# anxingle/AlphaPig

Hardware: AMD Instinct MI355X
Metric: self-play games/sec (15x15, n_playout=400) (higher is better)
Workload: dtype f32 (split operands on the bf16/fp16 matrix pipe, fp32 accumulate; <=1e-4 vs float64 oracle)

## Files before the change

### alphapig_amd/csrc/trunk15_wino3h16.h

```cpp
#pragma once
#include <hip/hip_runtime.h>

#include <cmath>
#include <cstdint>
#include <type_traits>

#include "trunk15_wino3h.h"

namespace apz {

struct Wino3H16 {
    static constexpr int C = 128, CK = 16, NCHUNK = C / CK;
    static constexpr int GPLANE = 240;
    static constexpr int VTERM = 32 * 32, VPOS = 2 * VTERM, V_BYTES = 36 * VPOS;
    static constexpr int UNIT = 2 * 32 * 16;
    static constexpr size_t UPK_BYTES = (size_t)4 * 4 * NCHUNK * 9 * 2 * UNIT;
    static constexpr int BIAS_FLOATS = 256;
    static constexpr int MQ_FLOATS = 36 * 16 * 32;
    static constexpr int SROW = 20, SPLANE = 16 * SROW;
    static constexpr int STG_FLOATS = 8 * 4 * SPLANE;
    static constexpr int LDS_BYTES = 2 * V_BYTES;
    static_assert((MQ_FLOATS + STG_FLOATS) * 4 <= LDS_BYTES, "the epilogue area fits over V");
    static_assert(LDS_BYTES <= 160 * 1024, "LDS");
    static_assert(UPK_BYTES == Wino3H::UPK_BYTES, "same weight buffer as trunk15_wino3h.h");
    __host__ __device__ static size_t upk_offset(int co, int ci, int pos, int term) {
        const int i = pos / 6, k = pos % 6, ri = i / 3, ki = k / 3, p9 = 3 * (i % 3) + (k % 3);
        const int cog = co >> 5, r = co & 31, chunk = ci >> 4, half = (ci >> 3) & 1, w = 2 * ri + ki;
        return ((((size_t)(cog * 4 + w) * NCHUNK + chunk) * 9 + p9) * 2 + term) * UNIT + half * 512 + r * 16 + (ci & 7) * 2;
    }
    static float scale_for(double m) { return Wino3H::scale_for(m); }
};

#ifdef APZ_WINO3H_STAMPS
__device__ unsigned long long apz_wino3h16_stamps[4 * 8 * 12];
#endif

#ifndef APZH16_RING
#define APZH16_RING 3
#endif
#ifndef APZH16_RAW_SLOT
#define APZH16_RAW_SLOT 4
#endif

enum { WINO3H16_PLAIN = 0, WINO3H16_STATS = 1, WINO3H16_DGRAD = 2, WINO3H16_PLAIN_SCALED = 3 };

constexpr int ACT_WINDOW_LOG2 = 4;
constexpr int ACT_EXP_MAX = 100;

inline int act_exponent_for(float m) {
    if (!(m > 0.f)) return 0;
    int ex;
    std::frexp((double)m, &ex);
    const int a = ACT_WINDOW_LOG2 - (ex - 1);
    return a < -ACT_EXP_MAX ? -ACT_EXP_MAX : (a > ACT_EXP_MAX ? ACT_EXP_MAX : a);
}

__device__ __forceinline__ int wino3h16_dgrad_exponent(float m) {
    if (!(m > 0.f)) return 0;
    const int e = (int)((__builtin_bit_cast(unsigned, m) >> 23) & 255u);
    const int a = 134 - e;
    return a < -64 ? -64 : (a > 110 ? 110 : a);
}

template <bool RESID, bool RELU = true, int FORM = WINO3H16_PLAIN>
__global__ __launch_bounds__(512) void trunk15_wino3h16_kernel(const float* __restrict__ in, const void* __restrict__ upk,
                                                               const float* __restrict__ bias, const float* __restrict__ resid,
                                                               float* __restrict__ out, int n, unsigned* __restrict__ flag,
                                                               void* __restrict__ aux, int aux_n) {
    using T = Wino3H16;
    constexpr bool STATS = FORM == WINO3H16_STATS, DGRAD = FORM == WINO3H16_DGRAD, SCALED = FORM == WINO3H16_PLAIN_SCALED;
    static_assert(FORM == WINO3H16_PLAIN || SCALED || !RELU, "the training forms have no ReLU");
    static_assert(!SCALED || RELU, "the scaled form is a self-play form");
    static_assert(!STATS || !RESID, "STATS: bias only");
#ifdef APZ_WINO3H_STAMPS
    unsigned long long st_acc[12] = {0, 0, 0, 0, 0, 0, 0, 0, 0, 0, 0, 0};
    unsigned long long st_t = __builtin_readcyclecounter();
    const unsigned long long st_t0 = st_t, st_r0 = __builtin_amdgcn_s_memrealtime();
#define APZH16_STAMP(ph_)                                             \
    {                                                                 \
        const unsigned long long now_ = __builtin_readcyclecounter(); \
        st_acc[ph_] += now_ - st_t;                                   \
        st_t = now_;                                                  \
    }
#else
#define APZH16_STAMP(ph_)
#endif
    extern __shared__ __attribute__((aligned(16))) float lds[];
    char* vbase = reinterpret_cast<char*>(lds);
    float* mq = lds;
    float* stg = mq + T::MQ_FLOATS;

    const int tid = threadIdx.x, lane = tid & 63;
    const int wave = __builtin_amdgcn_readfirstlane(tid >> 6);

    const int npairs = (n + 1) >> 1, G_ = (int)gridDim.x, b_ = (int)blockIdx.x;
    const bool duo = (G_ & 15) == 0;
    const int pair0 = duo ? ((b_ >> 4) * 8 + (b_ & 7)) : b_;
    const int pstride = duo ? (G_ >> 1) : G_;
    const int h_fix = (b_ >> 3) & 1;
    const int np = pair0 < npairs ? (npairs - pair0 + pstride - 1) / pstride : 0;
    const int nitems = duo ? np : 2 * np;
    if (np == 0) return;
    auto item_pair = [&](int t) { return pair0 + (duo ? t : (t >> 1)) * pstride; };
    auto item_half = [&](int t) { return duo ? h_fix : (t & 1); };

    float xsc = 1.f, xisc = 1.f;
    bool aux_inf = false;
    if constexpr (DGRAD) {
        const float* pm = static_cast<const float*>(aux);
        float m = 0.f;
        for (int i = tid; i < aux_n; i += 512) m = fmaxf(m, fabsf(pm[i]));
#pragma unroll
        for (int off = 32; off > 0; off >>= 1) m = fmaxf(m, __shfl_xor(m, off, 64));
        if (lane == 0) lds[wave] = m;
        __syncthreads();
#pragma unroll
        for (int w = 0; w < 8; w++) m = fmaxf(m, lds[w]);
        const int a = __builtin_amdgcn_readfirstlane(wino3h16_dgrad_exponent(m));
        aux_inf = !(m <= 3.4028234664e38f);
        xsc = __builtin_bit_cast(float, (unsigned)(127 + a) << 23);
        xisc = __builtin_bit_cast(float, (unsigned)(127 - a) << 23);
    }
    if constexpr (SCALED) {
        xsc = __builtin_bit_cast(float, (unsigned)(127 + aux_n) << 23);
        xisc = __builtin_bit_cast(float, (unsigned)(127 - aux_n) << 23);
    }

    const unsigned plane_b = T::GPLANE * 4;
    const unsigned act_bytes = (unsigned)n * T::C * plane_b;
    const __amdgpu_buffer_rsrc_t r_in = __builtin_amdgcn_make_buffer_rsrc(const_cast<float*>(in), 0, act_bytes, 0x00020000);
    const __amdgpu_buffer_rsrc_t r_res =
        __builtin_amdgcn_make_buffer_rsrc(const_cast<float*>(RESID ? resid : in), 0, act_bytes, 0x00020000);
    const __amdgpu_buffer_rsrc_t r_out = __builtin_amdgcn_make_buffer_rsrc(out, 0, act_bytes, 0x00020000);
    const __amdgpu_buffer_rsrc_t r_u =
        __builtin_amdgcn_make_buffer_rsrc(const_cast<void*>(upk), 0, (unsigned)T::UPK_BYTES, 0x00020000);
    const __amdgpu_buffer_rsrc_t r_st =
        __builtin_amdgcn_make_buffer_rsrc(STATS ? aux : out, 0, STATS ? (unsigned)n * T::C * 16u : 0u, 0x00020000);
    auto bload = [](const __amdgpu_buffer_rsrc_t& r, unsigned voff, unsigned soff) {
        return __builtin_bit_cast(f32x4, __builtin_amdgcn_raw_buffer_load_b128(r, voff, soff, 0));
    };
    auto bstore = [](const __amdgpu_buffer_rsrc_t& r, unsigned voff, unsigned soff, const f32x4 v) {
        __builtin_amdgcn_raw_buffer_store_b128(__builtin_bit_cast(u32x4, v), r, voff + soff, 0, 0);
    };

    const int tb = wave & 1, cq = wave >> 1;
    const int ttx = lane & 3, tty = (lane >> 2) & 3, tile = lane & 15, cpl = (lane >> 4) & 1, e = lane >> 5;
    const int chl = 4 * cq + 2 * cpl + e;
    const int cpair = 2 * cq + cpl;
    const int vcol = tb * 16 + tile;
    const int tv_off = vcol * 32 + (((cpair >> 2) ^ ((vcol >> 3) & 1)) * 16) + (cpair & 3) * 4 + e * 3 * T::VPOS;
    const unsigned col16_mask = ttx == 3 ? 0u : 0xffffffffu;
    const float c4l = ttx == 0 ? 0.f : 4.f;
    const unsigned raw_vo = (unsigned)(2 * cpl + e) * plane_b + (unsigned)(tty * 4 * 16 + ttx * 4) * 4;
    const unsigned raw_vo3 = tty == 3 ? 0x80000000u : raw_vo + 3u * 64u;
    f32x4 raw[4];
    auto raw_load = [&](int t, int c) {
        const int bdp = 2 * item_pair(t) + tb;
        const int bd = bdp < n ? bdp : n - 1;
        const unsigned so = (unsigned)(bd * T::C + c * T::CK + 4 * cq) * plane_b;
#pragma unroll
        for (int r = 0; r < 3; r++) raw[r] = bload(r_in, raw_vo + (unsigned)r * 64u, so);
        raw[3] = bload(r_in, raw_vo3, so);
    };

    f32x2 tt[6][2];
    float oo[6];
    auto vpass = [&](int kc) {
        f32x2 x[6];
#pragma unroll
        for (int j = 0; j < 2; j++) {
            const float r3 = raw[3][2 * kc + j], r0 = raw[0][2 * kc + j];
            x[0][j] = __builtin_bit_cast(float, __builtin_amdgcn_update_dpp(0, __builtin_bit_cast(int, r3), 0x114, 0xF, 0xF, true));
            x[5][j] = __builtin_bit_cast(float, __builtin_amdgcn_update_dpp(0, __builtin_bit_cast(int, r0), 0x104, 0xF, 0xF, true));
        }
#pragma unroll
        for (int r = 0; r < 4; r++) x[r + 1] = f32x2{raw[r][2 * kc], raw[r][2 * kc + 1]};
        const f32x2 a = fma2(-4.f, x[2], x[4]), b = fma2(-4.f, x[1], x[3]);
        const f32x2 c = x[4] - x[2], d = x[3] - x[1];
        tt[0][kc] = fma2(4.f, x[0], fma2(-5.f, x[2], x[4]));
        tt[1][kc] = a + b;
        tt[2][kc] = a - b;
        tt[3][kc] = fma2(2.f, d, c);
        tt[4][kc] = fma2(-2.f, d, c);
        tt[5][kc] = fma2(4.f, x[1], fma2(-5.f, x[3], x[5]));
    };
    auto col_pass = [&](int j) {
        const float c3 = tt[j][1][1], c0 = tt[j][0][0];
        const int l = __builtin_amdgcn_mov_dpp(__builtin_bit_cast(int, c3), 0x90, 0xF, 0xF, true);
        const int r = __builtin_amdgcn_mov_dpp(__builtin_bit_cast(int, c0), 0xF9, 0xF, 0xF, true);
        const float v0 = __builtin_bit_cast(float, l), v5 = __builtin_bit_cast(float, (unsigned)r & col16_mask);
        const f32x2 ab = fma2(-4.f, tt[j][0], tt[j][1]);
        const f32x2 dc = tt[j][1] - tt[j][0];
        oo[0] = __builtin_fmaf(c4l, v0, __builtin_fmaf(-5.f, tt[j][0][1], tt[j][1][1]));
        oo[3] = __builtin_fmaf(2.f, dc[0], dc[1]);
        oo[1] = ab[1] + ab[0];
        oo[4] = __builtin_fmaf(-2.f, dc[0], dc[1]);
        oo[2] = ab[1] - ab[0];
        oo[5] = __builtin_fmaf(4.f, tt[j][0][0], __builtin_fmaf(-5.f, tt[j][1][0], v5));
    };
    auto exchange = [&]() {
        asm("s_nop 1\n\tv_permlane32_swap_b32 %0, %3\n\tv_permlane32_swap_b32 %1, %4\n\tv_permlane32_swap_b32 %2, %5"
            : "+v"(oo[0]), "+v"(oo[1]), "+v"(oo[2]), "+v"(oo[3]), "+v"(oo[4]), "+v"(oo[5]));
    };
    auto emit = [&](char* vp, float ev, float od) {
        typedef _Float16 f16x2_ __attribute__((ext_vector_type(2)));
        const f16x2_ h2 = {(_Float16)ev, (_Float16)od};
        const unsigned hu = __builtin_bit_cast(unsigned, h2);
        unsigned lu;
        asm("v_fma_mixlo_f16 %0, %1, -1.0, %2 op_sel:[0,0,0] op_sel_hi:[1,0,0]" : "=v"(lu) : "v"(hu), "v"(ev));
        asm("v_fma_mixhi_f16 %0, %1, -1.0, %2 op_sel:[1,0,0] op_sel_hi:[1,0,0]" : "+v"(lu) : "v"(hu), "v"(od));
        *reinterpret_cast<unsigned*>(vp) = hu;
        *reinterpret_cast<unsigned*>(vp + T::VTERM) = lu;
    };
    auto tslice = [&](int vpar, auto KK) {
        constexpr int K = decltype(KK)::value;
        char* vp = vbase + vpar * T::V_BYTES + tv_off;
        if constexpr ((DGRAD || SCALED) && K == 0) {
#pragma unroll
            for (int r = 0; r < 4; r++) raw[r] *= xsc;
        }
        if constexpr (K < 2) vpass(K);
        else if constexpr (K >= 3) {
            constexpr int j = (K - 3) / 4, part = (K - 3) % 4;
            if constexpr (part == 0) col_pass(j);
            else if constexpr (part == 1) exchange();
            else if constexpr (part == 2) {
                emit(vp + (j * 6 + 0) * T::VPOS, oo[0], oo[3]);
                emit(vp + (j * 6 + 1) * T::VPOS, oo[1], oo[4]);
            } else emit(vp + (j * 6 + 2) * T::VPOS, oo[2], oo[5]);
        }
    };
    auto transform = [&](int vpar) {
#define APZH16_TS(k) tslice(vpar, std::integral_constant<int, k>{});
        APZH16_TS(0) APZH16_TS(1) APZH16_TS(2) APZH16_TS(3) APZH16_TS(4) APZH16_TS(5) APZH16_TS(6) APZH16_TS(7) APZH16_TS(8)
        APZH16_TS(9) APZH16_TS(10) APZH16_TS(11) APZH16_TS(12) APZH16_TS(13) APZH16_TS(14) APZH16_TS(15) APZH16_TS(16)
        APZH16_TS(17) APZH16_TS(18) APZH16_TS(19) APZH16_TS(20) APZH16_TS(21) APZH16_TS(22) APZH16_TS(23) APZH16_TS(24)
        APZH16_TS(25) APZH16_TS(26)
#undef APZH16_TS
    };

    const int cc = wave >> 2, ri = (wave >> 1) & 1, ki = wave & 1, blk = wave & 3;
    const int r31 = lane & 31, hh = lane >> 5;
    const unsigned a_vo = lane * 16;
    const int wpos0 = 18 * ri + 3 * ki;
    auto pos_off = [](int p9) { return (6 * (p9 / 3) + (p9 % 3)) * T::VPOS; };

    static constexpr int RING = APZH16_RING;
    static_assert(18 % RING == 0 && RING >= 2, "ring slots must tile two chunks");
    f16x8 ah[RING], al[RING];
    auto unit_base = [&](int t, int c) {
        const int cog = 2 * item_half(t) + cc;
        return (unsigned)(((cog * 4 + blk) * T::NCHUNK + c) * 18) * T::UNIT;
    };
    unsigned ub_cur = 0, ub_nxt = 0;
    auto unit_pair_at = [&](unsigned base, int p9, int slot) {
        const int u = 2 * p9;
        ah[slot] = __builtin_bit_cast(f16x8, __builtin_amdgcn_raw_buffer_load_b128(r_u, a_vo + (unsigned)(u & 3) * T::UNIT,
                                                                                  base + (unsigned)(u >> 2) * 4u * T::UNIT, 0));
        al[slot] = __builtin_bit_cast(f16x8, __builtin_amdgcn_raw_buffer_load_b128(r_u, a_vo + (unsigned)((u + 1) & 3) * T::UNIT,
                                                                                  base + (unsigned)((u + 1) >> 2) * 4u * T::UNIT, 0));
    };
    auto unit_load = [&](int p9, int slot) {
        if (p9 < 9) unit_pair_at(ub_cur, p9, slot);
        else unit_pair_at(ub_nxt, p9 - 9, slot);
    };

    unsigned nonfinite = aux_inf ? 1u : 0u;

    ub_cur = ub_nxt = unit_base(0, 0);
#pragma unroll
    for (int u = 0; u < RING - 1; u++) unit_load(u, u);
    raw_load(0, 0);
    if (wave >= 4) __builtin_amdgcn_s_setprio(1);

    for (int t = 0; t < nitems; t++) {
        const int h = item_half(t);
        const int bd0 = 2 * item_pair(t);
        const bool two = bd0 + 1 < n;
        __syncthreads();
        APZH16_STAMP(5)
        transform(0);
        raw_load(t, 1);
        f32x16h acc[9];
#pragma unroll
        for (int p = 0; p < 9; p++)
#pragma unroll
            for (int v = 0; v < 16; v++) acc[p][v] = 0.f;
        APZH16_STAMP(0)

        f16x8 bfr[2];
        auto chunk = [&](int c, auto PAR, auto XF, auto LD) {
            constexpr int par = decltype(PAR)::value;
            constexpr bool xf = decltype(XF)::value, ld = decltype(LD)::value;
            __syncthreads();
            APZH16_STAMP(1)
            ub_cur = ub_nxt;
            ub_nxt = c + 1 < T::NCHUNK ? ub_cur + 18u * T::UNIT : (t + 1 < nitems ? unit_base(t + 1, 0) : ub_cur + 18u * T::UNIT);
            const char* vp = vbase + par * T::V_BYTES;
            int le = __builtin_amdgcn_mbcnt_hi(~0u, __builtin_amdgcn_mbcnt_lo(~0u, 0u));
            asm volatile("" : "+v"(le));
            const int fcol = le & 31;
            const int b_hi = wpos0 * T::VPOS + fcol * 32 + ((((le >> 5) & 1) ^ ((fcol >> 3) & 1)) * 16);
            const int b_lo = b_hi + T::VTERM;
            bfr[0] = *reinterpret_cast<const f16x8*>(vp + b_hi);
            bfr[1] = *reinterpret_cast<const f16x8*>(vp + b_lo);
#define APZH16_SLOT(k)                                                                                                   \
            {                                                                                                            \
                constexpr int p9 = (k), slot = (par * 9 + (k)) % RING;                                                   \
                                                                   \
                acc[p9] = __builtin_amdgcn_mfma_f32_32x32x16_f16(ah[slot], bfr[1], acc[p9], 0, 0, 0);                    \
                if (p9 + 1 < 9) bfr[1] = *reinterpret_cast<const f16x8*>(vp + b_lo + pos_off(p9 + 1));                   \
                acc[p9] = __builtin_amdgcn_mfma_f32_32x32x16_f16(al[slot], bfr[0], acc[p9], 0, 0, 0);                    \
                acc[p9] = __builtin_amdgcn_mfma_f32_32x32x16_f16(ah[slot], bfr[0], acc[p9], 0, 0, 0);                    \
                if (p9 + 1 < 9) bfr[0] = *reinterpret_cast<const f16x8*>(vp + b_hi + pos_off(p9 + 1));                   \
                if (xf) {                                                                                                \
                    tslice(1 - par, std::integral_constant<int, 3 * (k)>{});                                             \
                    tslice(1 - par, std::integral_constant<int, 3 * (k) + 1>{});                                         \
                    tslice(1 - par, std::integral_constant<int, 3 * (k) + 2>{});                                         \
                }                                                                                                        \
                if ((k) == APZH16_RAW_SLOT && ld) raw_load(t, c + 2);                                                    \
                             \
                unit_load((k) + RING - 1, (par * 9 + (k) + RING - 1) % RING);                                            \
                __builtin_amdgcn_sched_barrier(0);                                                                       \
            }
            APZH16_SLOT(0) APZH16_SLOT(1) APZH16_SLOT(2) APZH16_SLOT(3) APZH16_SLOT(4) APZH16_SLOT(5) APZH16_SLOT(6) APZH16_SLOT(7) APZH16_SLOT(8)
#undef APZH16_SLOT
            APZH16_STAMP(2)
        };
        using P0 = std::integral_constant<int, 0>;
        using P1 = std::integral_constant<int, 1>;
        using Y = std::true_type;
        using N = std::false_type;
        for (int c = 0; c < T::NCHUNK - 2; c += 2) {
            chunk(c, P0{}, Y{}, Y{});
            chunk(c + 1, P1{}, Y{}, Y{});
        }
        chunk(T::NCHUNK - 2, P0{}, Y{}, N{});
        chunk(T::NCHUNK - 1, P1{}, N{}, N{});

        const int cosel = lane >> 5;
        const int col = lane & 31, gbd = col >> 4, gtile = col & 15;
        const int gty = gtile >> 2, gtx = gtile & 3;
        float* sw = stg + wave * (4 * T::SPLANE);
        const int s_lin = (lane >> 2) * T::SROW + (lane & 3) * 4;
        const unsigned ep_vo = lane < 60 ? lane * 16 : 0x80000000u;
        auto row_chan = [&](int s, int row) { return (2 * h + (row >> 3)) * 32 + 8 * s + (row & 7); };
        f32x4 rs[4];
        auto resid_request = [&](int s) {
#pragma unroll
            for (int pl = 0; pl < 4; pl++) {
                const int bdp = bd0 + (pl & 1);
                const int bd = bdp < n ? bdp : n - 1;
                rs[pl] = bload(r_res, ep_vo, (unsigned)(bd * T::C + row_chan(s, 2 * wave + (pl >> 1))) * plane_b);
            }
        };
        if (RESID) resid_request(0);
        auto ep_step = [&](auto S_) {
            constexpr int s = decltype(S_)::value;
            __syncthreads();
            APZH16_STAMP(4)
            {
                float* mw = mq + wpos0 * 512 + (8 * cc + 4 * hh) * 32 + r31;
#pragma unroll
                for (int p9 = 0; p9 < 9; p9++)
#pragma unroll
                    for (int e4 = 0; e4 < 4; e4++) mw[(6 * (p9 / 3) + p9 % 3) * 512 + e4 * 32] = acc[p9][4 * s + e4];
            }
            if (RESID) {
#pragma unroll
                for (int pl = 0; pl < 4; pl++) *reinterpret_cast<f32x4*>(sw + pl * T::SPLANE + s_lin) = rs[pl];
            }
            if (s == 3 && t + 1 < nitems) raw_load(t + 1, 0);
            APZH16_STAMP(8)
            __syncthreads();
            APZH16_STAMP(10)
            {
                const int co16 = 2 * wave + cosel;
                const float* mp = mq + co16 * 32 + col;
                float hrow[6][4];
#pragma unroll
                for (int i = 0; i < 6; i++) {
                    float m[6];
#pragma unroll
                    for (int k = 0; k < 6; k++) m[k] = mp[(6 * i + k) * 512];
                    const float s12 = m[1] + m[2], d12 = m[1] - m[2], s34 = m[3] + m[4], d34 = m[3] - m[4];
                    hrow[i][0] = (m[0] + s12) + s34;
                    hrow[i][1] = __builtin_fmaf(2.f, d34, d12);
                    hrow[i][2] = __builtin_fmaf(4.f, s34, s12);
                    hrow[i][3] = __builtin_fmaf(8.f, d34, d12) + m[5];
                }
                if (RESID && s + 1 < 4) resid_request(s + 1);
                const int ch = row_chan(s, co16);
                const float bv = bias[ch];
                const float is = (DGRAD || SCALED) ? bias[128 + ch] * xisc : bias[128 + ch];
                float* sp = sw + (cosel * 2 + gbd) * T::SPLANE + (4 * gty) * T::SROW + 4 * gtx;
                f32x4 y[4];
#pragma unroll
                for (int ee = 0; ee < 4; ee++) {
                    const float s12 = hrow[1][ee] + hrow[2][ee], d12 = hrow[1][ee] - hrow[2][ee];
                    const float s34 = hrow[3][ee] + hrow[4][ee], d34 = hrow[3][ee] - hrow[4][ee];
                    y[0][ee] = (hrow[0][ee] + s12) + s34;
                    y[1][ee] = __builtin_fmaf(2.f, d34, d12);
                    y[2][ee] = __builtin_fmaf(4.f, s34, s12);
                    y[3][ee] = __builtin_fmaf(8.f, d34, d12) + hrow[5][ee];
                }
                float chk = 0.f;
                float r1[4], r2[4];
#pragma unroll
                for (int a = 0; a < 4; a++) {
                    f32x4 v;
#pragma unroll
                    for (int ee = 0; ee < 4; ee++) v[ee] = __builtin_fmaf(y[a][ee], is, bv);
                    if (RESID) v += *reinterpret_cast<const f32x4*>(sp + a * T::SROW);
                    chk += (v[0] + v[1]) + (v[2] + v[3]);
#pragma unroll
                    for (int ee = 0; ee < 4; ee++) v[ee] = RELU ? fmaxf(v[ee], 0.f) : v[ee];
                    if (gtx == 3) v[3] = 0.f;
                    *reinterpret_cast<f32x4*>(sp + a * T::SROW) = v;
                    if constexpr (STATS) {
                        r1[a] = (v[0] + v[1]) + (v[2] + v[3]);
                        r2[a] = (v[0] * v[0] + v[1] * v[1]) + (v[2] * v[2] + v[3] * v[3]);
                    }
                }
                nonfinite |= ((chk - chk) != 0.f) ? 1u : 0u;
                if constexpr (STATS) {
                    if (gty == 3) r1[3] = 0.f, r2[3] = 0.f;
                    const double d1 = (double)wino3_row16_sum((r1[0] + r1[1]) + (r1[2] + r1[3]));
                    const double d2 = (double)wino3_row16_sum((r2[0] + r2[1]) + (r2[2] + r2[3]));
                    const bool mine = gtile == 0 && (gbd == 0 || two);
                    typedef double f64x2 __attribute__((ext_vector_type(2)));
                    const unsigned so = (unsigned)(ch * n + bd0 + gbd) * 16u;
                    bstore(r_st, mine ? so : 0x80000000u, 0u, __builtin_bit_cast(f32x4, f64x2{d1, d2}));
                }
            }
            APZH16_STAMP(9)
            wave_lds_fence();
#pragma unroll
            for (int pl = 0; pl < 4; pl++) {
                const f32x4 pv = *reinterpret_cast<const f32x4*>(sw + pl * T::SPLANE + s_lin);
                const unsigned vo = ((pl & 1) == 0 || two) ? ep_vo : 0x80000000u;
                bstore(r_out, vo, (unsigned)((bd0 + (pl & 1)) * T::C + row_chan(s, 2 * wave + (pl >> 1))) * plane_b, pv);
            }
            APZH16_STAMP(3)
        };
        ep_step(std::integral_constant<int, 0>{});
        ep_step(std::integral_constant<int, 1>{});
        ep_step(std::integral_constant<int, 2>{});
        ep_step(std::integral_constant<int, 3>{});
    }
    if (nonfinite && flag) *reinterpret_cast<volatile unsigned*>(flag) = 1u;
#ifdef APZ_WINO3H_STAMPS
    st_acc[7] = __builtin_readcyclecounter() - st_t0;
    st_acc[6] = __builtin_amdgcn_s_memrealtime() - st_r0;
    if (lane == 0 && blockIdx.x < 4)
        for (int i = 0; i < 12; i++) apz_wino3h16_stamps[(blockIdx.x * 8 + wave) * 12 + i] = st_acc[i];
#endif
#undef APZH16_STAMP
}

}
```

Measured before the change: 15.35.

## Overlap next item's input chunks with epilogue and store outputs directly from registers

The epilogue's M area moves to the second V buffer, so the first chunks of the next item can be transformed and loaded while the current item's epilogue runs. The per-item leading barrier and transform are hoisted into the chunk loop, and raw_load can address chunks past NCHUNK of the next item, using a zero-size resource for out-of-range prefetches. The LDS staging area for residual and output tiles is removed: residuals are loaded straight into registers and results are stored with buffer stores per tile row. This saves LDS round-trips and a fence, at the cost of less coalesced 16-byte global stores and more complex cross-item control flow.

Result: no change. 15.58 (median of 6 runs) (+1.5%).

```diff
diff --git a/alphapig_amd/csrc/trunk15_wino3h16.h b/alphapig_amd/csrc/trunk15_wino3h16.h
--- a/alphapig_amd/csrc/trunk15_wino3h16.h
+++ b/alphapig_amd/csrc/trunk15_wino3h16.h
@@ -17,10 +17,8 @@
     static constexpr size_t UPK_BYTES = (size_t)4 * 4 * NCHUNK * 9 * 2 * UNIT;
     static constexpr int BIAS_FLOATS = 256;
     static constexpr int MQ_FLOATS = 36 * 16 * 32;
-    static constexpr int SROW = 20, SPLANE = 16 * SROW;
-    static constexpr int STG_FLOATS = 8 * 4 * SPLANE;
     static constexpr int LDS_BYTES = 2 * V_BYTES;
-    static_assert((MQ_FLOATS + STG_FLOATS) * 4 <= LDS_BYTES, "the epilogue area fits over V");
+    static_assert(MQ_FLOATS * 4 <= V_BYTES, "the epilogue's M fits over one V buffer");
     static_assert(LDS_BYTES <= 160 * 1024, "LDS");
     static_assert(UPK_BYTES == Wino3H::UPK_BYTES, "same weight buffer as trunk15_wino3h.h");
     __host__ __device__ static size_t upk_offset(int co, int ci, int pos, int term) {
@@ -87,8 +85,7 @@
 #endif
     extern __shared__ __attribute__((aligned(16))) float lds[];
     char* vbase = reinterpret_cast<char*>(lds);
-    float* mq = lds;
-    float* stg = mq + T::MQ_FLOATS;
+    float* mq = lds + T::V_BYTES / 4;
 
     const int tid = threadIdx.x, lane = tid & 63;
     const int wave = __builtin_amdgcn_readfirstlane(tid >> 6);
@@ -128,7 +125,6 @@
 
     const unsigned plane_b = T::GPLANE * 4;
     const unsigned act_bytes = (unsigned)n * T::C * plane_b;
-    const __amdgpu_buffer_rsrc_t r_in = __builtin_amdgcn_make_buffer_rsrc(const_cast<float*>(in), 0, act_bytes, 0x00020000);
     const __amdgpu_buffer_rsrc_t r_res =
         __builtin_amdgcn_make_buffer_rsrc(const_cast<float*>(RESID ? resid : in), 0, act_bytes, 0x00020000);
     const __amdgpu_buffer_rsrc_t r_out = __builtin_amdgcn_make_buffer_rsrc(out, 0, act_bytes, 0x00020000);
@@ -155,12 +151,15 @@
     const unsigned raw_vo3 = tty == 3 ? 0x80000000u : raw_vo + 3u * 64u;
     f32x4 raw[4];
     auto raw_load = [&](int t, int c) {
+        const bool real = c <= T::NCHUNK;
+        if (c >= T::NCHUNK) t += 1, c -= T::NCHUNK;
         const int bdp = 2 * item_pair(t) + tb;
         const int bd = bdp < n ? bdp : n - 1;
         const unsigned so = (unsigned)(bd * T::C + c * T::CK + 4 * cq) * plane_b;
-#pragma unroll
-        for (int r = 0; r < 3; r++) raw[r] = bload(r_in, raw_vo + (unsigned)r * 64u, so);
-        raw[3] = bload(r_in, raw_vo3, so);
+        const __amdgpu_buffer_rsrc_t r = __builtin_amdgcn_make_buffer_rsrc(const_cast<float*>(in), 0, real ? act_bytes : 0u, 0x00020000);
+#pragma unroll
+        for (int rr = 0; rr < 3; rr++) raw[rr] = bload(r, raw_vo + (unsigned)rr * 64u, so);
+        raw[3] = bload(r, raw_vo3, so);
     };
 
     f32x2 tt[6][2];
@@ -277,10 +276,13 @@
         const int h = item_half(t);
         const int bd0 = 2 * item_pair(t);
         const bool two = bd0 + 1 < n;
-        __syncthreads();
-        APZH16_STAMP(5)
-        transform(0);
-        raw_load(t, 1);
+        const bool has_next = t + 1 < nitems;
+        if (t == 0) {
+            __syncthreads();
+            APZH16_STAMP(5)
+            transform(0);
+            raw_load(0, 1);
+        }
         f32x16h acc[9];
 #pragma unroll
         for (int p = 0; p < 9; p++)
@@ -331,30 +333,31 @@
         using P1 = std::integral_constant<int, 1>;
         using Y = std::true_type;
         using N = std::false_type;
-        for (int c = 0; c < T::NCHUNK - 2; c += 2) {
+        static_assert(T::NCHUNK % 2 == 0, "chunk 0 of every item in V[0], M over V[1]");
+        const int cend = has_next ? T::NCHUNK : T::NCHUNK - 2;
+        for (int c = 0; c < cend; c += 2) {
             chunk(c, P0{}, Y{}, Y{});
             chunk(c + 1, P1{}, Y{}, Y{});
         }
-        chunk(T::NCHUNK - 2, P0{}, Y{}, N{});
-        chunk(T::NCHUNK - 1, P1{}, N{}, N{});
+        if (!has_next) {
+            chunk(T::NCHUNK - 2, P0{}, Y{}, N{});
+            chunk(T::NCHUNK - 1, P1{}, N{}, N{});
+        }
 
         const int cosel = lane >> 5;
         const int col = lane & 31, gbd = col >> 4, gtile = col & 15;
         const int gty = gtile >> 2, gtx = gtile & 3;
-        float* sw = stg + wave * (4 * T::SPLANE);
-        const int s_lin = (lane >> 2) * T::SROW + (lane & 3) * 4;
-        const unsigned ep_vo = lane < 60 ? lane * 16 : 0x80000000u;
         auto row_chan = [&](int s, int row) { return (2 * h + (row >> 3)) * 32 + 8 * s + (row & 7); };
+        const unsigned ep_tile = (unsigned)cosel * plane_b + (unsigned)(4 * gty * 16 + 4 * gtx) * 4;
+        const unsigned ep_ld = ep_tile + ((gbd && two) ? (unsigned)T::C * plane_b : 0u);
+        const unsigned ep_st = (gbd && !two) ? 0x80000000u : ep_tile + (unsigned)gbd * T::C * plane_b;
+        auto ep_row = [&](unsigned base, int a) { return (a == 3 && gty == 3) ? 0x80000000u : base + (unsigned)a * 64u; };
+        auto ep_so = [&](int s) { return (unsigned)(bd0 * T::C + row_chan(s, 2 * wave)) * plane_b; };
         f32x4 rs[4];
-        auto resid_request = [&](int s) {
-#pragma unroll
-            for (int pl = 0; pl < 4; pl++) {
-                const int bdp = bd0 + (pl & 1);
-                const int bd = bdp < n ? bdp : n - 1;
-                rs[pl] = bload(r_res, ep_vo, (unsigned)(bd * T::C + row_chan(s, 2 * wave + (pl >> 1))) * plane_b);
-            }
-        };
-        if (RESID) resid_request(0);
+        if (RESID) {
+#pragma unroll
+            for (int a = 0; a < 4; a++) rs[a] = bload(r_res, ep_row(ep_ld, a), ep_so(0));
+        }
         auto ep_step = [&](auto S_) {
             constexpr int s = decltype(S_)::value;
             __syncthreads();
@@ -366,11 +369,7 @@
 #pragma unroll
                     for (int e4 = 0; e4 < 4; e4++) mw[(6 * (p9 / 3) + p9 % 3) * 512 + e4 * 32] = acc[p9][4 * s + e4];
             }
-            if (RESID) {
-#pragma unroll
-                for (int pl = 0; pl < 4; pl++) *reinterpret_cast<f32x4*>(sw + pl * T::SPLANE + s_lin) = rs[pl];
-            }
-            if (s == 3 && t + 1 < nitems) raw_load(t + 1, 0);
+            if (s == 3 && has_next) raw_load(t + 1, 1);
             APZH16_STAMP(8)
             __syncthreads();
             APZH16_STAMP(10)
@@ -389,11 +388,10 @@
                     hrow[i][2] = __builtin_fmaf(4.f, s34, s12);
                     hrow[i][3] = __builtin_fmaf(8.f, d34, d12) + m[5];
                 }
-                if (RESID && s + 1 < 4) resid_request(s + 1);
                 const int ch = row_chan(s, co16);
                 const float bv = bias[ch];
                 const float is = (DGRAD || SCALED) ? bias[128 + ch] * xisc : bias[128 + ch];
-                float* sp = sw + (cosel * 2 + gbd) * T::SPLANE + (4 * gty) * T::SROW + 4 * gtx;
+                const unsigned so = ep_so(s);
                 f32x4 y[4];
 #pragma unroll
                 for (int ee = 0; ee < 4; ee++) {
@@ -411,37 +409,35 @@
                     f32x4 v;
 #pragma unroll
                     for (int ee = 0; ee < 4; ee++) v[ee] = __builtin_fmaf(y[a][ee], is, bv);
-                    if (RESID) v += *reinterpret_cast<const f32x4*>(sp + a * T::SROW);
+                    if (RESID) {
+                        v += rs[a];
+                    }
                     chk += (v[0] + v[1]) + (v[2] + v[3]);
 #pragma unroll
                     for (int ee = 0; ee < 4; ee++) v[ee] = RELU ? fmaxf(v[ee], 0.f) : v[ee];
                     if (gtx == 3) v[3] = 0.f;
-                    *reinterpret_cast<f32x4*>(sp + a * T::SROW) = v;
+                    bstore(r_out, ep_row(ep_st, a), so, v);
                     if constexpr (STATS) {
                         r1[a] = (v[0] + v[1]) + (v[2] + v[3]);
                         r2[a] = (v[0] * v[0] + v[1] * v[1]) + (v[2] * v[2] + v[3] * v[3]);
                     }
                 }
                 nonfinite |= ((chk - chk) != 0.f) ? 1u : 0u;
+                if (RESID && s + 1 < 4) {
+#pragma unroll
+                    for (int a = 0; a < 4; a++) rs[a] = bload(r_res, ep_row(ep_ld, a), ep_so(s + 1));
+                }
                 if constexpr (STATS) {
                     if (gty == 3) r1[3] = 0.f, r2[3] = 0.f;
                     const double d1 = (double)wino3_row16_sum((r1[0] + r1[1]) + (r1[2] + r1[3]));
                     const double d2 = (double)wino3_row16_sum((r2[0] + r2[1]) + (r2[2] + r2[3]));
                     const bool mine = gtile == 0 && (gbd == 0 || two);
                     typedef double f64x2 __attribute__((ext_vector_type(2)));
-                    const unsigned so = (unsigned)(ch * n + bd0 + gbd) * 16u;
-                    bstore(r_st, mine ? so : 0x80000000u, 0u, __builtin_bit_cast(f32x4, f64x2{d1, d2}));
+                    const unsigned sto = (unsigned)(ch * n + bd0 + gbd) * 16u;
+                    bstore(r_st, mine ? sto : 0x80000000u, 0u, __builtin_bit_cast(f32x4, f64x2{d1, d2}));
                 }
             }
             APZH16_STAMP(9)
-            wave_lds_fence();
-#pragma unroll
-            for (int pl = 0; pl < 4; pl++) {
-                const f32x4 pv = *reinterpret_cast<const f32x4*>(sw + pl * T::SPLANE + s_lin);
-                const unsigned vo = ((pl & 1) == 0 || two) ? ep_vo : 0x80000000u;
-                bstore(r_out, vo, (unsigned)((bd0 + (pl & 1)) * T::C + row_chan(s, 2 * wave + (pl >> 1))) * plane_b, pv);
-            }
-            APZH16_STAMP(3)
         };
         ep_step(std::integral_constant<int, 0>{});
         ep_step(std::integral_constant<int, 1>{});
```
